# DocF/multispectral-object-detection

Measured on AMD Instinct MI355X. Metric: image-pairs/sec fwd, yolov5l+CFTx3 640×640 bs64, 1/2/4/8 GPU, higher is better.
Workload: dtype bf16; 1 GPU; cfg3 (yolov5l_fusion_transformerx3_FLIR_aligned) two-stream forward, 640x640, 64 pairs/GPU, BN folded, pre-NMS detections; pairs_per_gpu=64, image_size=640, parallelism=batch-shard x1, hip_graph=True, two_hip_streams=False, forwards_in_flight=3, streams_per_forward_in_flight=1, single_in_flight_streams=2

## Files before the change

### multispectral-object-detection_amd/csrc/attention.hip

```cpp
#include "cft_common.h"

template <typename T>
__global__ void __launch_bounds__(256) attention_kernel(const unsigned char* __restrict__ qkv, unsigned char* __restrict__ out,
                                                        int heads, int dkp, float scale, uint32_t drop_thresh, float inv_keep,
                                                        unsigned long long seed) {
  constexpr int GE = Elem<T>::GE;
  constexpr int ES = (int)sizeof(T);
  constexpr int T_TOK = 128;
  constexpr int KT = GE / 4;
  constexpr int NCH = 8 / KT;
  constexpr int PS_B = T_TOK * ES + 16;
  extern __shared__ __attribute__((aligned(16))) unsigned char smem[];
  const int KS_B = dkp * ES + 16;
  unsigned char* sK = smem;
  unsigned char* sVT = smem + T_TOK * KS_B;

  const int b = blockIdx.x / heads, head = blockIdx.x % heads;
  const int tid = threadIdx.x, lane = tid & 63, wave = tid >> 6;
  const int lrow = lane & 15, lgrp = lane >> 4;
  const int G = dkp / GE;
  const long ldq_b = (long)3 * heads * dkp * ES;
  const long ldo_b = (long)heads * dkp * ES;
  const unsigned char* qbase = qkv + (long)b * T_TOK * ldq_b + (long)head * dkp * ES;
  const unsigned char* kbase = qbase + (long)heads * dkp * ES;
  const unsigned char* vbase = kbase + (long)heads * dkp * ES;

#define ATT_STAGE_VT(c0_, cw_)                                                                             \
  {                                                                                                        \
    const int cg_ = (cw_) / GE;                                                                            \
    for (int i = tid; i < T_TOK * cg_; i += 256) {                                                         \
      const int t = i / cg_, kg = i - t * cg_;                                                             \
      const gran_t g = *reinterpret_cast<const gran_t*>(vbase + t * ldq_b + (long)((c0_) + kg * GE) * ES); \
      if (ES == 2) {                                                                                       \
        _Pragma("unroll") for (int e = 0; e < 4; ++e) {                                                    \
          *reinterpret_cast<uint16_t*>(sVT + (kg * GE + 2 * e) * PS_B + t * 2) = (uint16_t)(g[e] & 0xffffu); \
          *reinterpret_cast<uint16_t*>(sVT + (kg * GE + 2 * e + 1) * PS_B + t * 2) = (uint16_t)(g[e] >> 16); \
        }                                                                                                  \
      } else {                                                                                             \
        _Pragma("unroll") for (int e = 0; e < 4; ++e)                                                      \
          *reinterpret_cast<uint32_t*>(sVT + (kg * GE + e) * PS_B + t * 4) = g[e];                         \
      }                                                                                                    \
    }                                                                                                      \
  }

  for (int i = tid; i < T_TOK * G; i += 256) {
    const int t = i / G, kg = i - t * G;
    *reinterpret_cast<gran_t*>(sK + t * KS_B + kg * 16) = *reinterpret_cast<const gran_t*>(kbase + t * ldq_b + kg * 16);
  }
  {
    const int cw0 = dkp < 64 ? dkp : 64;
    ATT_STAGE_VT(0, cw0)
  }
  __syncthreads();

  f32x4_t s[2][8];
#pragma unroll
  for (int i = 0; i < 2; ++i)
#pragma unroll
    for (int j = 0; j < 8; ++j) s[i][j] = f32x4_t{0.f, 0.f, 0.f, 0.f};
  const int ksteps = G >> 2;
  for (int ks = 0; ks < ksteps; ++ks) {
    const int kg = ks * 4 + lgrp;
    gran_t qf[2];
#pragma unroll
    for (int i = 0; i < 2; ++i)
      qf[i] = *reinterpret_cast<const gran_t*>(qbase + (long)(wave * 32 + i * 16 + lrow) * ldq_b + kg * 16);
#pragma unroll
    for (int j = 0; j < 8; ++j) {
      const gran_t kf = *reinterpret_cast<const gran_t*>(sK + (j * 16 + lrow) * KS_B + kg * 16);
#pragma unroll
      for (int i = 0; i < 2; ++i) s[i][j] = mma_granule<T>(kf, qf[i], s[i][j]);
    }
  }

  float inv_sum[2];
  gran_t pf[2][NCH];
#pragma unroll
  for (int i = 0; i < 2; ++i) {
    float mx = -INFINITY;
#pragma unroll
    for (int j = 0; j < 8; ++j)
#pragma unroll
      for (int e = 0; e < 4; ++e) { s[i][j][e] *= scale; mx = fmaxf(mx, s[i][j][e]); }
    mx = fmaxf(mx, __shfl_xor(mx, 16));
    mx = fmaxf(mx, __shfl_xor(mx, 32));
    float sum = 0.f;
#pragma unroll
    for (int j = 0; j < 8; ++j)
#pragma unroll
      for (int e = 0; e < 4; ++e) { const float pv = __expf(s[i][j][e] - mx); s[i][j][e] = pv; sum += pv; }
    sum += __shfl_xor(sum, 16);
    sum += __shfl_xor(sum, 32);
    inv_sum[i] = 1.0f / sum;
    if (drop_thresh != 0u) {
      const unsigned long long qrow = ((unsigned long long)blockIdx.x * T_TOK + (wave * 32 + i * 16 + lrow)) * T_TOK;
#pragma unroll
      for (int j = 0; j < 8; ++j)
#pragma unroll
        for (int e = 0; e < 4; ++e)
          s[i][j][e] = cft_hash32(seed, qrow + (unsigned)(j * 16 + lgrp * 4 + e)) >= drop_thresh ? s[i][j][e] * inv_keep : 0.0f;
    }
#pragma unroll
    for (int c = 0; c < NCH; ++c) {
      if constexpr (ES == 2) {
        typedef Elem<typename Half16<T>::type> E16;
        pf[i][c] = gran_t{E16::pack2(s[i][2 * c][0], s[i][2 * c][1]), E16::pack2(s[i][2 * c][2], s[i][2 * c][3]),
                          E16::pack2(s[i][2 * c + 1][0], s[i][2 * c + 1][1]), E16::pack2(s[i][2 * c + 1][2], s[i][2 * c + 1][3])};
      } else {
        pf[i][c] = gran_t{__float_as_uint(s[i][c][0]), __float_as_uint(s[i][c][1]), __float_as_uint(s[i][c][2]), __float_as_uint(s[i][c][3])};
      }
    }
  }

  for (int c0 = 0; c0 < dkp; c0 += 64) {
    const int cw = (dkp - c0) < 64 ? (dkp - c0) : 64;
    if (c0 > 0) {
      __syncthreads();
      ATT_STAGE_VT(c0, cw)
      __syncthreads();
    }
    const int ntc = cw >> 4;
    f32x4_t o[2][4];
#pragma unroll
    for (int i = 0; i < 2; ++i)
#pragma unroll
      for (int j = 0; j < 4; ++j) o[i][j] = f32x4_t{0.f, 0.f, 0.f, 0.f};
#pragma unroll
    for (int c = 0; c < NCH; ++c) {
#pragma unroll
      for (int j = 0; j < 4; ++j) {
        if (j < ntc) {
          const unsigned char* vrow = sVT + (j * 16 + lrow) * PS_B;
          gran_t vf;
          if constexpr (ES == 2) {
            const uint2 lo = *reinterpret_cast<const uint2*>(vrow + ((2 * c) * 16 + lgrp * 4) * 2);
            const uint2 hi = *reinterpret_cast<const uint2*>(vrow + ((2 * c + 1) * 16 + lgrp * 4) * 2);
            vf = gran_t{lo.x, lo.y, hi.x, hi.y};
          } else {
            vf = *reinterpret_cast<const gran_t*>(vrow + (c * 16 + lgrp * 4) * 4);
          }
#pragma unroll
          for (int i = 0; i < 2; ++i) o[i][j] = mma_granule<T>(vf, pf[i][c], o[i][j]);
        }
      }
    }
#pragma unroll
    for (int i = 0; i < 2; ++i)
#pragma unroll
      for (int j = 0; j < 4; ++j) {
        if (j < ntc) {
          const int row = wave * 32 + i * 16 + lrow;
          float v[4];
#pragma unroll
          for (int e = 0; e < 4; ++e) v[e] = o[i][j][e] * inv_sum[i];
          unsigned char* dst = out + ((long)b * T_TOK + row) * ldo_b + ((long)head * dkp + c0 + j * 16 + lgrp * 4) * ES;
          if constexpr (ES == 2) {
            typedef Elem<typename Half16<T>::type> E16;
            *reinterpret_cast<uint2*>(dst) = uint2{E16::pack2(v[0], v[1]), E16::pack2(v[2], v[3])};
          }
          else *reinterpret_cast<f32x4_t*>(dst) = f32x4_t{v[0], v[1], v[2], v[3]};
        }
      }
  }
#undef ATT_STAGE_VT
}

extern "C" int cft_attention(const void* qkv, void* out, int B, int heads, int dk, int dkp,
                             int dtype, float attn_pdrop, unsigned long long seed, void* stream) {
  CFT_REQUIRE(qkv && out, "cft_attention: null pointer");
  CFT_REQUIRE(attn_pdrop >= 0.0f && attn_pdrop < 1.0f, "cft_attention: attn_pdrop must be in [0, 1) (0 = inference)");
  CFT_REQUIRE(cft_is_dtype(dtype), "cft_attention: bad dtype");
  const int es = cft_elem_size(dtype);
  const int kstep = es == 2 ? 32 : 16;
  CFT_REQUIRE(B > 0 && heads > 0 && dk > 0 && dkp >= dk && dkp % kstep == 0 && dkp <= 256, "cft_attention: dkp must be a multiple of 32 (bf16, f16) / 16 (f32), >= dk, <= 256");
  const int ps = 128 * es + 16, ks = dkp * es + 16;
  const size_t smem = (size_t)128 * ks + (size_t)64 * ps;
  CFT_REQUIRE(smem <= 160 * 1024, "cft_attention: head too wide for LDS");
  const float scale = 1.0f / sqrtf((float)dk);
  CFT_DISPATCH_DTYPE(dtype, T, {
    cft_allow_lds<&attention_kernel<T>>(160 * 1024);
    hipLaunchKernelGGL(attention_kernel<T>, dim3(B * heads), dim3(256), smem, as_stream(stream), (const unsigned char*)qkv, (unsigned char*)out, heads, dkp, scale,
                       (uint32_t)((double)attn_pdrop * 4294967296.0), 1.0f / (1.0f - attn_pdrop), seed);
  });
  return cft_check_launch("attention_kernel");
}
```

### multispectral-object-detection_amd/csrc/pointwise.hip

```cpp
#include "cft_common.h"
#include "resize_common.h"

static inline int grid_for(long work, int block) {
  long g = (work + block - 1) / block;
  const long cap = 256L * 16;
  return (int)(g < 1 ? 1 : (g > cap ? cap : g));
}

template <typename T>
__global__ void __launch_bounds__(256) focus_s2d_kernel(const float* __restrict__ in, unsigned char* __restrict__ out,
                                                        int B, int H, int W) {
  const int Ho = H >> 1, Wo = W >> 1;
  const long total = (long)B * Ho * Wo;
  for (long idx = (long)blockIdx.x * blockDim.x + threadIdx.x; idx < total; idx += (long)gridDim.x * blockDim.x) {
    const int x = (int)(idx % Wo);
    const long t = idx / Wo;
    const int y = (int)(t % Ho);
    const int b = (int)(t / Ho);
    float v[16];
#pragma unroll
    for (int c = 0; c < 3; ++c) {
      const float* base = in + (((long)b * 3 + c) * H + 2 * y) * W + 2 * x;
      const float2 top = *reinterpret_cast<const float2*>(base);
      const float2 bot = *reinterpret_cast<const float2*>(base + W);
      v[0 + c] = top.x;
      v[3 + c] = bot.x;
      v[6 + c] = top.y;
      v[9 + c] = bot.y;
    }
    v[12] = v[13] = v[14] = v[15] = 0.f;
    constexpr int GE = Elem<T>::GE;
    gran_t* o = reinterpret_cast<gran_t*>(out + idx * 16 * sizeof(T));
#pragma unroll
    for (int k = 0; k < 16 / GE; ++k) o[k] = Elem<T>::pack(v + k * GE);
  }
}

extern "C" int cft_focus_s2d(const float* in, void* out, int B, int H, int W, int dtype, void* stream) {
  CFT_REQUIRE(in && out, "cft_focus_s2d: null pointer");
  CFT_REQUIRE(B > 0 && H > 0 && W > 0 && (H % 2 == 0) && (W % 2 == 0), "cft_focus_s2d: H and W must be even");
  CFT_REQUIRE(cft_is_dtype(dtype), "cft_focus_s2d: bad dtype");
  const long total = (long)B * (H / 2) * (W / 2);
  const int grid = grid_for(total, 256);
  CFT_DISPATCH_DTYPE(dtype, T, hipLaunchKernelGGL(focus_s2d_kernel<T>, dim3(grid), dim3(256), 0, as_stream(stream), in, (unsigned char*)out, B, H, W));
  return cft_check_launch("focus_s2d_kernel");
}

template <typename T>
__global__ void __launch_bounds__(256) focus_s2d_u8_kernel(const unsigned char* __restrict__ in, long sb, long sc, long sh,
                                                           unsigned char* __restrict__ out, int B, int H, int W, float scale) {
  const int Ho = H >> 1, Wo = W >> 1;
  const long total = (long)B * Ho * Wo;
  for (long idx = (long)blockIdx.x * blockDim.x + threadIdx.x; idx < total; idx += (long)gridDim.x * blockDim.x) {
    const int x = (int)(idx % Wo);
    const long t = idx / Wo;
    const int y = (int)(t % Ho);
    const int b = (int)(t / Ho);
    float v[16];
#pragma unroll
    for (int c = 0; c < 3; ++c) {
      const unsigned char* base = in + (long)b * sb + (long)c * sc + (long)(2 * y) * sh + 2 * x;
      v[0 + c] = (float)base[0] * scale;
      v[6 + c] = (float)base[1] * scale;
      v[3 + c] = (float)base[sh] * scale;
      v[9 + c] = (float)base[sh + 1] * scale;
    }
    v[12] = v[13] = v[14] = v[15] = 0.f;
    constexpr int GE = Elem<T>::GE;
    gran_t* o = reinterpret_cast<gran_t*>(out + idx * 16 * sizeof(T));
#pragma unroll
    for (int k = 0; k < 16 / GE; ++k) o[k] = Elem<T>::pack(v + k * GE);
  }
}

extern "C" int cft_focus_s2d_u8(const unsigned char* in, long stride_b, long stride_c, long stride_h, void* out,
                                int B, int H, int W, float scale, int dtype, void* stream) {
  CFT_REQUIRE(in && out, "cft_focus_s2d_u8: null pointer");
  CFT_REQUIRE(B > 0 && H > 0 && W > 0 && (H % 2 == 0) && (W % 2 == 0), "cft_focus_s2d_u8: H and W must be even");
  CFT_REQUIRE(cft_is_dtype(dtype), "cft_focus_s2d_u8: bad dtype");
  CFT_REQUIRE(stride_h >= W && stride_c > 0 && stride_b > 0, "cft_focus_s2d_u8: bad strides");
  const long total = (long)B * (H / 2) * (W / 2);
  const int grid = grid_for(total, 256);
  CFT_DISPATCH_DTYPE(dtype, T, hipLaunchKernelGGL(focus_s2d_u8_kernel<T>, dim3(grid), dim3(256), 0, as_stream(stream), in, stride_b, stride_c, stride_h, (unsigned char*)out, B, H, W, scale));
  return cft_check_launch("focus_s2d_u8_kernel");
}

template <typename T>
__device__ __forceinline__ void gmax(float* a, const gran_t& g) {
  float f[Elem<T>::GE];
  Elem<T>::unpack(g, f);
// ... 15 lines not shown
  const long pix_stride = (long)ld * sizeof(T);
  for (int i = threadIdx.x; i < HW; i += blockDim.x) plane[i] = *reinterpret_cast<const gran_t*>(base + i * pix_stride);
  __syncthreads();
  const int rad[3] = {r1, r2, r3};
  for (int i = threadIdx.x; i < HW; i += blockDim.x) {
    const int y = i / W, x = i - y * W;
    float m[GE];
#pragma unroll
    for (int e = 0; e < GE; ++e) m[e] = -INFINITY;
    int done = -1;
#pragma unroll
    for (int k = 0; k < 3; ++k) {
      for (int d = done + 1; d <= rad[k]; ++d) {
        if (d == 0) { gmax<T>(m, plane[i]); continue; }
        if (x - d >= 0) gmax<T>(m, plane[i - d]);
        if (x + d < W) gmax<T>(m, plane[i + d]);
      }
      done = rad[k];
      rowm[k * HW + i] = Elem<T>::pack(m);
    }
  }
  __syncthreads();
  for (int i = threadIdx.x; i < HW; i += blockDim.x) {
    const int y = i / W;
#pragma unroll
    for (int k = 0; k < 3; ++k) {
      float m[GE];
#pragma unroll
      for (int e = 0; e < GE; ++e) m[e] = -INFINITY;
      const gran_t* src = rowm + k * HW;
      for (int d = -rad[k]; d <= rad[k]; ++d)
        if ((unsigned)(y + d) < (unsigned)H) gmax<T>(m, src[i + d * W]);
      *reinterpret_cast<gran_t*>(base + i * pix_stride + (long)(k + 1) * C * sizeof(T)) = Elem<T>::pack(m);
    }
  }
}

template <typename T>
__global__ void __launch_bounds__(512) spp_chain_kernel(unsigned char* buf, int H, int W, int C, int ld, int r, int G) {
  constexpr int GE = Elem<T>::GE;
  extern __shared__ __attribute__((aligned(16))) unsigned char smem[];
  const int HW = H * W, n = HW * G;
  gran_t* A = reinterpret_cast<gran_t*>(smem);
  gran_t* Bp = A + n;
  const int groups = (C / GE) / G;
  const int b = blockIdx.x / groups, g0 = (blockIdx.x - b * groups) * G;
  unsigned char* base = buf + ((long)b * HW * ld + (long)g0 * GE) * sizeof(T);
  const long pix_stride = (long)ld * sizeof(T);
  for (int i = threadIdx.x; i < n; i += blockDim.x) {
    const int px = i / G, g = i - px * G;
    A[i] = *reinterpret_cast<const gran_t*>(base + px * pix_stride + g * 16);
  }
  __syncthreads();
  for (int k = 0; k < 3; ++k) {
    for (int i = threadIdx.x; i < n; i += blockDim.x) {
      const int px = i / G;
      const int x = px % W;
      float m[GE];
      Elem<T>::unpack(A[i], m);
      for (int d = 1; d <= r; ++d) {
        if (x - d >= 0) gmax<T>(m, A[i - d * G]);
        if (x + d < W) gmax<T>(m, A[i + d * G]);
      }
      Bp[i] = Elem<T>::pack(m);
    }
    __syncthreads();
    for (int i = threadIdx.x; i < n; i += blockDim.x) {
      const int px = i / G, g = i - px * G;
      const int y = px / W;
      float m[GE];
      Elem<T>::unpack(Bp[i], m);
      for (int d = 1; d <= r; ++d) {
        if (y - d >= 0) gmax<T>(m, Bp[i - d * W * G]);
        if (y + d < H) gmax<T>(m, Bp[i + d * W * G]);
      }
      const gran_t o = Elem<T>::pack(m);
      A[i] = o;
      *reinterpret_cast<gran_t*>(base + px * pix_stride + ((long)(k + 1) * C * sizeof(T)) + g * 16) = o;
    }
    __syncthreads();
  }
}

extern "C" int cft_spp_maxpool(void* buf, int B, int H, int W, int C, int ld, int k1, int k2, int k3,
                               int dtype, void* stream) {
  CFT_REQUIRE(buf != nullptr, "cft_spp_maxpool: null pointer");
  CFT_REQUIRE(cft_is_dtype(dtype), "cft_spp_maxpool: bad dtype");
  const int ge = cft_granule(dtype);
  CFT_REQUIRE(C % ge == 0 && ld % ge == 0 && ld >= 4 * C, "cft_spp_maxpool: C/ld not granule aligned or ld < 4C");
  CFT_REQUIRE((k1 & 1) && (k2 & 1) && (k3 & 1) && k1 <= k2 && k2 <= k3 && k3 <= 13 && k1 >= 1, "cft_spp_maxpool: kernel sizes must be odd, ascending, <= 13");
  const int r1 = k1 / 2, r2 = k2 / 2, r3 = k3 / 2, gpc = C / ge;
  if (r1 >= 1 && r2 == 2 * r1 && r3 == 3 * r1 && (size_t)2 * H * W * 16 <= 160 * 1024) {
    int G = 1;
    for (int g = 4; g > 1; g >>= 1)
      if (gpc % g == 0 && (size_t)2 * H * W * g * 16 <= 64 * 1024) { G = g; break; }
    const size_t smem = (size_t)2 * H * W * G * 16;
    const int grid = B * (gpc / G);
    CFT_DISPATCH_DTYPE(dtype, T, {
      cft_allow_lds<&spp_chain_kernel<T>>(160 * 1024);
      hipLaunchKernelGGL(spp_chain_kernel<T>, dim3(grid), dim3(512), smem, as_stream(stream), (unsigned char*)buf, H, W, C, ld, r1, G);
    });
    return cft_check_launch("spp_chain_kernel");
  }
  const size_t smem = (size_t)4 * H * W * 16;
  CFT_REQUIRE(smem <= 160 * 1024, "cft_spp_maxpool: feature map too large for the LDS plane (H*W <= 2560)");
  const int grid = B * gpc;
  CFT_DISPATCH_DTYPE(dtype, T, {
    cft_allow_lds<&spp_maxpool_kernel<T>>(160 * 1024);
    hipLaunchKernelGGL(spp_maxpool_kernel<T>, dim3(grid), dim3(256), smem, as_stream(stream), (unsigned char*)buf, H, W, C, ld, r1, r2, r3);
  });
  return cft_check_launch("spp_maxpool_kernel");
}

__global__ void __launch_bounds__(256) copy_channels_kernel(const unsigned char* __restrict__ in, long ldi_b, long ioff_b,
                                                            unsigned char* __restrict__ out, long ldo_b, long ooff_b,
                                                            int B, int Ho, int Wo, int gpp, int up) {
  const long total = (long)B * Ho * Wo * gpp;
  const int Hi = Ho >> up, Wi = Wo >> up;
  for (long idx = (long)blockIdx.x * blockDim.x + threadIdx.x; idx < total; idx += (long)gridDim.x * blockDim.x) {
    const int gidx = (int)(idx % gpp);
    long t = idx / gpp;
    const int x = (int)(t % Wo); t /= Wo;
    const int y = (int)(t % Ho);
    const int b = (int)(t / Ho);
    const long ipix = ((long)b * Hi + (y >> up)) * Wi + (x >> up);
    const long opix = ((long)b * Ho + y) * Wo + x;
    *reinterpret_cast<gran_t*>(out + opix * ldo_b + ooff_b + gidx * 16L) =
        *reinterpret_cast<const gran_t*>(in + ipix * ldi_b + ioff_b + gidx * 16L);
  }
}

extern "C" int cft_copy_channels(const void* in, int ldi, int ioff, void* out, int ldo, int ooff,
                                 int B, int Ho, int Wo, int C, int up, int dtype, void* stream) {
  CFT_REQUIRE(in && out, "cft_copy_channels: null pointer");
  CFT_REQUIRE(cft_is_dtype(dtype), "cft_copy_channels: bad dtype");
  const int ge = cft_granule(dtype), es = cft_elem_size(dtype);
  CFT_REQUIRE(C % ge == 0 && ldi % ge == 0 && ioff % ge == 0 && ldo % ge == 0 && ooff % ge == 0, "cft_copy_channels: not granule aligned");
  CFT_REQUIRE(up >= 0 && up <= 3 && (Ho % (1 << up) == 0) && (Wo % (1 << up) == 0), "cft_copy_channels: bad upsample shift");
  const int gpp = C / ge;
  const long total = (long)B * Ho * Wo * gpp;
  hipLaunchKernelGGL(copy_channels_kernel, dim3(grid_for(total, 256)), dim3(256), 0, as_stream(stream),
                     (const unsigned char*)in, (long)ldi * es, (long)ioff * es, (unsigned char*)out, (long)ldo * es, (long)ooff * es,
                     B, Ho, Wo, gpp, up);
  return cft_check_launch("copy_channels_kernel");
}

template <typename TI, typename TO>
__global__ void __launch_bounds__(256) to_nhwc_kernel(const unsigned char* __restrict__ in, long sb, long sc, long sh, long sw,
                                                      unsigned char* __restrict__ out, long ldo_b, long ooff_b,
                                                      int B, int C, int H, int W, int gpp) {
  constexpr int GE = Elem<TO>::GE;
  const long total = (long)B * H * W * gpp;
  for (long idx = (long)blockIdx.x * blockDim.x + threadIdx.x; idx < total; idx += (long)gridDim.x * blockDim.x) {
    const int gidx = (int)(idx % gpp);
    long t = idx / gpp;
    const int x = (int)(t % W); t /= W;
    const int y = (int)(t % H);
    const int b = (int)(t / H);
    float v[GE];
#pragma unroll
    for (int e = 0; e < GE; ++e) {
      const int c = gidx * GE + e;
      float f = 0.0f;
      if (c < C) {
        const long o = (long)b * sb + (long)c * sc + (long)y * sh + (long)x * sw;
        if constexpr (sizeof(TI) == 4) f = reinterpret_cast<const float*>(in)[o];
        else {
          float lo, hi;
          Elem<TI>::unpack2((uint32_t)reinterpret_cast<const uint16_t*>(in)[o], lo, hi);
          f = lo;
        }
      }
      v[e] = f;
    }
    *reinterpret_cast<gran_t*>(out + (((long)b * H + y) * W + x) * ldo_b + ooff_b + gidx * 16L) = Elem<TO>::pack(v);
  }
}

extern "C" int cft_to_nhwc(const void* in, int in_dtype, long stride_b, long stride_c, long stride_h, long stride_w,
                           void* out, int ldo, int ooff, int B, int C, int cpad, int H, int W, int dtype, void* stream) {
// ... 5 lines not shown
  CFT_REQUIRE(ldo % ge == 0 && ooff % ge == 0 && ldo >= ooff + cpad, "cft_to_nhwc: output ld/offset not granule aligned or too small");
  const int gpp = cpad / ge;
  const long total = (long)B * H * W * gpp;
  const int grid = grid_for(total, 256);
  CFT_DISPATCH_DTYPE(in_dtype, TI, CFT_DISPATCH_DTYPE(dtype, TO,
      hipLaunchKernelGGL((to_nhwc_kernel<TI, TO>), dim3(grid), dim3(256), 0, as_stream(stream), (const unsigned char*)in, stride_b, stride_c, stride_h, stride_w,
                         (unsigned char*)out, (long)ldo * es, (long)ooff * es, B, C, H, W, gpp)));
  return cft_check_launch("to_nhwc_kernel");
}

template <typename T>
__global__ void __launch_bounds__(256) add_kernel(const unsigned char* a, long lda_b, long aoff_b,
                                                  const unsigned char* b, long ldb_b, long boff_b,
                                                  unsigned char* out, long ldo_b, long ooff_b, long M, int gpp) {
  constexpr int GE = Elem<T>::GE;
  const long total = M * gpp;
  for (long idx = (long)blockIdx.x * blockDim.x + threadIdx.x; idx < total; idx += (long)gridDim.x * blockDim.x) {
    const long m = idx / gpp;
    const long go = (idx - m * gpp) * 16L;
    float fa[GE], fb[GE];
    Elem<T>::unpack(*reinterpret_cast<const gran_t*>(a + m * lda_b + aoff_b + go), fa);
    Elem<T>::unpack(*reinterpret_cast<const gran_t*>(b + m * ldb_b + boff_b + go), fb);
#pragma unroll
    for (int e = 0; e < GE; ++e) fa[e] += fb[e];
    *reinterpret_cast<gran_t*>(out + m * ldo_b + ooff_b + go) = Elem<T>::pack(fa);
  }
}

extern "C" int cft_add(const void* a, int lda, int aoff, const void* b, int ldb, int boff,
                       void* out, int ldo, int ooff, long M, int C, int dtype, void* stream) {
  CFT_REQUIRE(a && b && out, "cft_add: null pointer");
  CFT_REQUIRE(cft_is_dtype(dtype), "cft_add: bad dtype");
  const int ge = cft_granule(dtype), es = cft_elem_size(dtype);
  CFT_REQUIRE(C % ge == 0 && lda % ge == 0 && aoff % ge == 0 && ldb % ge == 0 && boff % ge == 0 && ldo % ge == 0 && ooff % ge == 0,
              "cft_add: not granule aligned");
  const int gpp = C / ge;
  const int grid = grid_for(M * gpp, 256);
  CFT_DISPATCH_DTYPE(dtype, T, hipLaunchKernelGGL(add_kernel<T>, dim3(grid), dim3(256), 0, as_stream(stream), (const unsigned char*)a, (long)lda * es, (long)aoff * es,
                                                   (const unsigned char*)b, (long)ldb * es, (long)boff * es, (unsigned char*)out, (long)ldo * es, (long)ooff * es, M, gpp));
  return cft_check_launch("add_kernel");
}

static int cft_fail(const char* who, const char* what) {
  char buf[256];
  snprintf(buf, sizeof(buf), "%s: %s", who, what);
  cft_set_error(buf);
  return CFT_EINVAL;
}
#define CFT_REQUIRE_WHO(cond, what) \
  do {                              \
    if (!(cond)) return cft_fail(who, what); \
  } while (0)

#define CFT_GRID_RULE "anchor grid must satisfy 1 <= va, ha and va * ha <= 1024"
static inline bool cft_grid_ok(int va, int ha) { return va >= 1 && ha >= 1 && va * ha <= 1024; }

struct ChanRef {
  const void* p;
  int ld, off;
  bool aligned(int ge) const { return p == nullptr || (ld % ge == 0 && off % ge == 0); }
  unsigned char* ptr() const { return (unsigned char*)p; }
};

template <typename T, int VA, int HA>
__global__ void __launch_bounds__(256) gpt_tokenize_kernel(const unsigned char* rgb, long ld_rgb_b, long off_rgb_b,
                                                           const unsigned char* ir, long ld_ir_b, long off_ir_b,
                                                           const float* __restrict__ pos_emb, float* __restrict__ tokens,
                                                           int H, int W, int C, int va_arg, int ha_arg) {
  constexpr int GE = Elem<T>::GE;
  const int va = VA ? VA : va_arg, ha = HA ? HA : ha_arg;
  const int ncell = va * ha, ntok = 2 * ncell;
  const int b = blockIdx.x / ntok, cell = blockIdx.x - b * ntok;
  const int s = cell >= ncell ? 1 : 0, r = cell - s * ncell;
  const int i = r / ha, j = r - i * ha;
  const int h0 = (i * H) / va, h1 = ((i + 1) * H + va - 1) / va;
  const int w0 = (j * W) / ha, w1 = ((j + 1) * W + ha - 1) / ha;
  const unsigned char* src = s ? ir : rgb;
  const long ldb = s ? ld_ir_b : ld_rgb_b, offb = s ? off_ir_b : off_rgb_b;
  const float inv = 1.0f / (float)((h1 - h0) * (w1 - w0));
  for (int cg = threadIdx.x; cg < C / GE; cg += blockDim.x) {
    float acc[GE];
#pragma unroll
    for (int e = 0; e < GE; ++e) acc[e] = 0.f;
    for (int y = h0; y < h1; ++y)
      for (int x = w0; x < w1; ++x) {
        float f[GE];
        Elem<T>::unpack(*reinterpret_cast<const gran_t*>(src + (((long)b * H + y) * W + x) * ldb + offb + cg * 16L), f);
#pragma unroll
        for (int e = 0; e < GE; ++e) acc[e] += f[e];
      }
    float* o = tokens + ((long)b * ntok + cell) * C + cg * GE;
    const float* pe = pos_emb + (long)cell * C + cg * GE;
#pragma unroll
    for (int e = 0; e < GE; ++e) o[e] = acc[e] * inv + pe[e];
  }
}

template <int VA, int HA>
static int gpt_tokenize_launch(const char* who, ChanRef rgb, ChanRef ir, const float* pos_emb, float* tokens,
                               int B, int H, int W, int C, int va, int ha, int dtype, void* stream) {
  CFT_REQUIRE_WHO(rgb.p && ir.p && pos_emb && tokens, "null pointer");
  CFT_REQUIRE_WHO(cft_is_dtype(dtype), "bad dtype");
  const int ge = cft_granule(dtype);
  const long es = cft_elem_size(dtype);
  CFT_REQUIRE_WHO(C % ge == 0 && rgb.aligned(ge) && ir.aligned(ge), "not granule aligned");
  CFT_REQUIRE_WHO(B > 0 && H >= 1 && W >= 1, "bad shape");
  if constexpr (VA == 0) {
    CFT_REQUIRE_WHO(cft_grid_ok(va, ha), CFT_GRID_RULE);
    CFT_REQUIRE_WHO((long)B * 2 * va * ha < (1L << 31), "too many tokens");
  }
  int threads = C / ge;
  threads = threads < 64 ? 64 : (threads > 256 ? 256 : ((threads + 63) / 64) * 64);
  CFT_DISPATCH_DTYPE(dtype, T, hipLaunchKernelGGL((gpt_tokenize_kernel<T, VA, HA>), dim3(B * 2 * va * ha), dim3(threads), 0, as_stream(stream),
                                                   rgb.ptr(), rgb.ld * es, rgb.off * es, ir.ptr(), ir.ld * es, ir.off * es, pos_emb, tokens, H, W, C, va, ha));
  return cft_check_launch("gpt_tokenize_kernel");
}

extern "C" int cft_gpt_tokenize(const void* rgb, int ld_rgb, int off_rgb, const void* ir, int ld_ir, int off_ir,
                                const float* pos_emb, float* tokens, int B, int H, int W, int C,
                                int dtype, void* stream) {
  return gpt_tokenize_launch<8, 8>("cft_gpt_tokenize", {rgb, ld_rgb, off_rgb}, {ir, ld_ir, off_ir}, pos_emb, tokens, B, H, W, C, 8, 8, dtype, stream);
}

extern "C" int cft_gpt_tokenize_grid(const void* rgb, int ld_rgb, int off_rgb, const void* ir, int ld_ir, int off_ir,
                                     const float* pos_emb, float* tokens, int B, int H, int W, int C, int va, int ha,
                                     int dtype, void* stream) {
  return gpt_tokenize_launch<0, 0>("cft_gpt_tokenize_grid", {rgb, ld_rgb, off_rgb}, {ir, ld_ir, off_ir}, pos_emb, tokens, B, H, W, C, va, ha, dtype, stream);
}

template <int MAXV, bool REDUCE>
__global__ void __launch_bounds__(256) layernorm_kernel(float* __restrict__ x, const float* __restrict__ gamma, const float* __restrict__ beta,
                                                        unsigned char* __restrict__ y, long rows, int C, float eps, int out_dtype,
                                                        const float* __restrict__ parts, int nparts, long part_stride) {
  const int lane = threadIdx.x & 63;
  const long row = (long)blockIdx.x * 4 + (threadIdx.x >> 6);
  if (row >= rows) return;
  const int nv = C >> 2;
  float4* xr = reinterpret_cast<float4*>(x + row * C);
  float4 v[MAXV];
  float s = 0.f;
#pragma unroll
  for (int k = 0; k < MAXV; ++k) {
    const int idx = lane + k * 64;
    v[k] = make_float4(0.f, 0.f, 0.f, 0.f);
    if (idx < nv) {
      float4 a = xr[idx];
      if constexpr (REDUCE) {
        for (int sp = 0; sp < nparts; ++sp) {
          const float4 q = reinterpret_cast<const float4*>(parts + sp * part_stride + row * C)[idx];
          a.x += q.x; a.y += q.y; a.z += q.z; a.w += q.w;
        }
        xr[idx] = a;
      }
      v[k] = a;
    }
    s += v[k].x + v[k].y + v[k].z + v[k].w;
  }
#pragma unroll
  for (int o = 32; o > 0; o >>= 1) s += __shfl_xor(s, o);
  const float mean = s / (float)C;
  float q = 0.f;
#pragma unroll
  for (int k = 0; k < MAXV; ++k) {
    const int idx = lane + k * 64;
    if (idx < nv) {
      const float a = v[k].x - mean, b = v[k].y - mean, c = v[k].z - mean, d = v[k].w - mean;
      q += a * a + b * b + c * c + d * d;
    }
  }
#pragma unroll
  for (int o = 32; o > 0; o >>= 1) q += __shfl_xor(q, o);
  const float rstd = rsqrtf(q / (float)C + eps);
#pragma unroll
// ... 115 lines not shown
          for (int e = 0; e < GE; ++e) v0[e] += v1[e];
          *reinterpret_cast<gran_t*>(sum + pix * lds_b + soff_b + cb) = Elem<T>::pack(v0);
        }
      } else {
#pragma unroll
        for (int e = 0; e < GE; ++e) v0[e] += hx * r0[e] + lx * r1[e];
        *reinterpret_cast<gran_t*>(out0 + pix * ldo0_b + ooff0_b + cb) = Elem<T>::pack(v0);
      }
    }
  }
}

static inline int gpt_upsample_grid_chunk(int C, int ha, int ns) {
  int cw = (16 * 1024) / (ns * ha);
  cw -= cw % 8;
  return C < cw ? C : cw;
}

template <bool DUAL, int VA, int HA>
static int gpt_upsample_launch(const char* who, const float* tokens, int s, ChanRef base0, ChanRef base1, ChanRef out0, ChanRef out1, ChanRef sum,
                               int B, int H, int W, int C, int va, int ha, int dtype, void* stream) {
  constexpr int NS = DUAL ? 2 : 1;
  const int ge = cft_granule(dtype);
  const long es = cft_elem_size(dtype);
  CFT_REQUIRE_WHO(C % ge == 0 && base0.aligned(ge) && base1.aligned(ge) && out0.aligned(ge) && out1.aligned(ge) && sum.aligned(ge), "not granule aligned");
  int cw = C;
  if constexpr (VA != 0) {
    CFT_REQUIRE_WHO(C % 4 == 0 && (long)B * H < (1L << 31), "C must be a multiple of 4");
    CFT_REQUIRE_WHO((size_t)NS * HA * C * sizeof(float) <= (size_t)NS * 64 * 1024,
                    DUAL ? "C too large for the LDS rows (C <= 2048)" : "C too large for the LDS row (C <= 2048)");
  } else {
    CFT_REQUIRE_WHO(C % 4 == 0 && C <= 2048 && B > 0 && H >= 1 && W >= 1 && (long)B * H < (1L << 31), "C must be a multiple of 4, <= 2048");
    cw = gpt_upsample_grid_chunk(C, ha, NS);
  }
  const size_t smem = (size_t)NS * ha * cw * sizeof(float);
  CFT_DISPATCH_DTYPE(dtype, T, {
    if constexpr (DUAL && VA != 0) cft_allow_lds<&gpt_upsample_kernel<T, DUAL, VA, HA>>(128 * 1024);
    hipLaunchKernelGGL((gpt_upsample_kernel<T, DUAL, VA, HA>), dim3(B * H), dim3(256), smem, as_stream(stream), tokens, s,
                       base0.ptr(), base0.ld * es, base0.off * es, base1.ptr(), base1.ld * es, base1.off * es,
                       out0.ptr(), out0.ld * es, out0.off * es, out1.ptr(), out1.ld * es, out1.off * es,
                       sum.ptr(), sum.ld * es, sum.off * es, B, H, W, C, va, ha, cw);
  });
  return cft_check_launch("gpt_upsample_kernel");
}

extern "C" int cft_gpt_upsample_add(const float* tokens, int s, const void* base, int ldb, int boff,
                                    void* out, int ldo, int ooff, int B, int H, int W, int C,
                                    int dtype, void* stream) {
  CFT_REQUIRE(tokens && out, "cft_gpt_upsample_add: null pointer");
  CFT_REQUIRE(cft_is_dtype(dtype), "cft_gpt_upsample_add: bad dtype");
  CFT_REQUIRE(s == 0 || s == 1, "cft_gpt_upsample_add: stream index must be 0 or 1");
  return gpt_upsample_launch<false, 8, 8>("cft_gpt_upsample_add", tokens, s, {base, ldb, boff}, {}, {out, ldo, ooff}, {}, {}, B, H, W, C, 8, 8, dtype, stream);
}

extern "C" int cft_gpt_upsample_add2(const float* tokens, const void* base0, int ldb0, int boff0, const void* base1, int ldb1, int boff1,
                                     void* out0, int ldo0, int ooff0, void* out1, int ldo1, int ooff1, void* sum, int lds, int soff,
                                     int B, int H, int W, int C, int dtype, void* stream) {
  CFT_REQUIRE(tokens && base0 && base1 && out0 && out1, "cft_gpt_upsample_add2: null pointer");
  CFT_REQUIRE(cft_is_dtype(dtype), "cft_gpt_upsample_add2: bad dtype");
  return gpt_upsample_launch<true, 8, 8>("cft_gpt_upsample_add2", tokens, 0, {base0, ldb0, boff0}, {base1, ldb1, boff1}, {out0, ldo0, ooff0},
                                         {out1, ldo1, ooff1}, {sum, lds, soff}, B, H, W, C, 8, 8, dtype, stream);
}

extern "C" int cft_gpt_upsample_add_grid(const float* tokens, int s, const void* base, int ldb, int boff,
                                         void* out, int ldo, int ooff, int B, int H, int W, int C, int va, int ha,
                                         int dtype, void* stream) {
  CFT_REQUIRE(tokens && out, "cft_gpt_upsample_add_grid: null pointer");
  CFT_REQUIRE(cft_is_dtype(dtype), "cft_gpt_upsample_add_grid: bad dtype");
  CFT_REQUIRE(s == 0 || s == 1, "cft_gpt_upsample_add_grid: stream index must be 0 or 1");
  CFT_REQUIRE(cft_grid_ok(va, ha), "cft_gpt_upsample_add_grid: " CFT_GRID_RULE);
  return gpt_upsample_launch<false, 0, 0>("cft_gpt_upsample_add_grid", tokens, s, {base, ldb, boff}, {}, {out, ldo, ooff}, {}, {}, B, H, W, C, va, ha, dtype, stream);
}

extern "C" int cft_gpt_upsample_add2_grid(const float* tokens, const void* base0, int ldb0, int boff0, const void* base1, int ldb1, int boff1,
                                          void* out0, int ldo0, int ooff0, void* out1, int ldo1, int ooff1, void* sum, int lds, int soff,
                                          int B, int H, int W, int C, int va, int ha, int dtype, void* stream) {
  CFT_REQUIRE(tokens && base0 && base1 && out0 && out1, "cft_gpt_upsample_add2_grid: null pointer");
  CFT_REQUIRE(cft_is_dtype(dtype), "cft_gpt_upsample_add2_grid: bad dtype");
  CFT_REQUIRE(cft_grid_ok(va, ha), "cft_gpt_upsample_add2_grid: " CFT_GRID_RULE);
  return gpt_upsample_launch<true, 0, 0>("cft_gpt_upsample_add2_grid", tokens, 0, {base0, ldb0, boff0}, {base1, ldb1, boff1}, {out0, ldo0, ooff0},
                                         {out1, ldo1, ooff1}, {sum, lds, soff}, B, H, W, C, va, ha, dtype, stream);
}

__global__ void __launch_bounds__(256) detect_decode_kernel(const float* __restrict__ logits, int ldl, float* __restrict__ raw,
                                                            float* __restrict__ pred, const float* __restrict__ anchors,
                                                            int B, int ny, int nx, int na, int no, float stride,
                                                            long row0, long total_rows) {
  const long total = (long)B * na * ny * nx * no;
  for (long idx = (long)blockIdx.x * blockDim.x + threadIdx.x; idx < total; idx += (long)gridDim.x * blockDim.x) {
    const int o = (int)(idx % no);
    long t = idx / no;
    const int x = (int)(t % nx); t /= nx;
    const int y = (int)(t % ny); t /= ny;
    const int a = (int)(t % na);
    const int b = (int)(t / na);
    const float v = logits[(((long)b * ny + y) * nx + x) * ldl + a * no + o];
    raw[idx] = v;
    const float sg = 1.0f / (1.0f + __expf(-v));
    float r;
    if (o == 0) r = (sg * 2.0f - 0.5f + (float)x) * stride;
    else if (o == 1) r = (sg * 2.0f - 0.5f + (float)y) * stride;
    else if (o < 4) { const float w = sg * 2.0f; r = w * w * anchors[a * 2 + (o - 2)]; }
    else r = sg;
    pred[((long)b * total_rows + row0 + ((long)a * ny + y) * nx + x) * no + o] = r;
  }
}

extern "C" int cft_detect_decode(const float* logits, int ldl, float* raw, float* pred, const float* anchors,
                                 int B, int ny, int nx, int na, int no, float stride,
                                 long row0, long total_rows, void* stream) {
  CFT_REQUIRE(logits && raw && pred && anchors, "cft_detect_decode: null pointer");
  CFT_REQUIRE(B > 0 && ny > 0 && nx > 0 && na > 0 && no >= 5 && ldl >= na * no, "cft_detect_decode: bad shape");
  CFT_REQUIRE(row0 >= 0 && row0 + (long)na * ny * nx <= total_rows, "cft_detect_decode: rows out of range");
  const long total = (long)B * na * ny * nx * no;
  hipLaunchKernelGGL(detect_decode_kernel, dim3(grid_for(total, 256)), dim3(256), 0, as_stream(stream), logits, ldl, raw, pred, anchors,
                     B, ny, nx, na, no, stride, row0, total_rows);
  return cft_check_launch("detect_decode_kernel");
}

__global__ void __launch_bounds__(256) letterbox_u8_kernel(const unsigned char* __restrict__ src, int sh, int sw, long src_row_stride,
                                                           unsigned char* __restrict__ dst, int dh, int dw, long dsy, long dsx, long dsc, int flip,
                                                           int rh, int rw, int top, int left, int c0, int c1, int c2) {
  const long total = (long)dh * dw;
  const double scale_x = cft_linear_scale(rw, sw), scale_y = cft_linear_scale(rh, sh);
  const bool resize = rh != sh || rw != sw;
  for (long idx = (long)blockIdx.x * blockDim.x + threadIdx.x; idx < total; idx += (long)gridDim.x * blockDim.x) {
    const int y = (int)(idx / dw), x = (int)(idx - (long)y * dw);
    const int ry = y - top, rx = x - left;
    int v[3] = {c0, c1, c2};
    if (ry >= 0 && ry < rh && rx >= 0 && rx < rw) {
      if (!resize) {
        const unsigned char* s = src + (long)ry * src_row_stride + rx * 3L;
        v[0] = s[0]; v[1] = s[1]; v[2] = s[2];
      } else {
        const CftLinearTap tx = cft_linear_tap_x(rx, scale_x, sw), ty = cft_linear_tap_y(ry, scale_y, sh);
        const unsigned char* r0 = src + (long)ty.s0 * src_row_stride;
        const unsigned char* r1 = src + (long)ty.s1 * src_row_stride;
#pragma unroll
        for (int c = 0; c < 3; ++c)
          v[c] = cft_linear_blend(r0[tx.s0 * 3 + c], r0[tx.s1 * 3 + c], r1[tx.s0 * 3 + c], r1[tx.s1 * 3 + c], tx, ty);
      }
    }
#pragma unroll
    for (int c = 0; c < 3; ++c) {
      int o = v[c];
      o = o < 0 ? 0 : (o > 255 ? 255 : o);
      dst[(long)y * dsy + (long)x * dsx + (long)(flip ? 2 - c : c) * dsc] = (unsigned char)o;
    }
  }
}

extern "C" int cft_letterbox_u8(const unsigned char* src, int src_h, int src_w, long src_row_stride,
                                unsigned char* dst, int dst_h, int dst_w, long dst_stride_y, long dst_stride_x, long dst_stride_c, int flip_channels,
                                int resized_h, int resized_w, int top, int left, int color0, int color1, int color2, void* stream) {
  CFT_REQUIRE(src && dst, "cft_letterbox_u8: null pointer");
  CFT_REQUIRE(src_h > 0 && src_w > 0 && dst_h > 0 && dst_w > 0 && resized_h > 0 && resized_w > 0, "cft_letterbox_u8: non-positive size");
  CFT_REQUIRE(top >= 0 && left >= 0 && top + resized_h <= dst_h && left + resized_w <= dst_w, "cft_letterbox_u8: the resized image does not fit the destination");
  CFT_REQUIRE(src_row_stride >= 3L * src_w, "cft_letterbox_u8: bad source row stride");
  const long total = (long)dst_h * dst_w;
  hipLaunchKernelGGL(letterbox_u8_kernel, dim3(grid_for(total, 256)), dim3(256), 0, as_stream(stream), src, src_h, src_w, src_row_stride,
                     dst, dst_h, dst_w, dst_stride_y, dst_stride_x, dst_stride_c, flip_channels, resized_h, resized_w, top, left, color0, color1, color2);
  return cft_check_launch("letterbox_u8_kernel");
}
```

Measured before the change: 3702 image-pairs/sec.

## Specialize attention staging, add SPP r2 kernel, vectorize detect decode and pooling

Measured after the change: 3722 image-pairs/sec, median of 5. About the same (+0.6%).

```diff
diff --git a/multispectral-object-detection_amd/csrc/attention.hip b/multispectral-object-detection_amd/csrc/attention.hip
--- a/multispectral-object-detection_amd/csrc/attention.hip
+++ b/multispectral-object-detection_amd/csrc/attention.hip
@@ -1,6 +1,6 @@
 #include "cft_common.h"
 
-template <typename T>
+template <typename T, int GC>
 __global__ void __launch_bounds__(256) attention_kernel(const unsigned char* __restrict__ qkv, unsigned char* __restrict__ out,
                                                         int heads, int dkp, float scale, uint32_t drop_thresh, float inv_keep,
                                                         unsigned long long seed) {
@@ -18,12 +18,28 @@
   const int b = blockIdx.x / heads, head = blockIdx.x % heads;
   const int tid = threadIdx.x, lane = tid & 63, wave = tid >> 6;
   const int lrow = lane & 15, lgrp = lane >> 4;
-  const int G = dkp / GE;
+  const int G = GC ? GC : dkp / GE;
+  constexpr int CG0 = GC * GE < 64 ? GC : 64 / GE;
+  constexpr int KIT = GC / 2, VIT = CG0 / 2;
+  constexpr int QST = GC / 4;
   const long ldq_b = (long)3 * heads * dkp * ES;
   const long ldo_b = (long)heads * dkp * ES;
   const unsigned char* qbase = qkv + (long)b * T_TOK * ldq_b + (long)head * dkp * ES;
   const unsigned char* kbase = qbase + (long)heads * dkp * ES;
   const unsigned char* vbase = kbase + (long)heads * dkp * ES;
+
+#define ATT_SCATTER_VT(g_, t_, kg_)                                                                          \
+  {                                                                                                          \
+    if (ES == 2) {                                                                                           \
+      _Pragma("unroll") for (int e = 0; e < 4; ++e) {                                                        \
+        *reinterpret_cast<uint16_t*>(sVT + ((kg_) * GE + 2 * e) * PS_B + (t_) * 2) = (uint16_t)((g_)[e] & 0xffffu); \
+        *reinterpret_cast<uint16_t*>(sVT + ((kg_) * GE + 2 * e + 1) * PS_B + (t_) * 2) = (uint16_t)((g_)[e] >> 16); \
+      }                                                                                                      \
+    } else {                                                                                                 \
+      _Pragma("unroll") for (int e = 0; e < 4; ++e)                                                          \
+        *reinterpret_cast<uint32_t*>(sVT + ((kg_) * GE + e) * PS_B + (t_) * 4) = (g_)[e];                    \
+    }                                                                                                        \
+  }
 
 #define ATT_STAGE_VT(c0_, cw_)                                                                             \
   {                                                                                                        \
@@ -31,27 +47,55 @@
     for (int i = tid; i < T_TOK * cg_; i += 256) {                                                         \
       const int t = i / cg_, kg = i - t * cg_;                                                             \
       const gran_t g = *reinterpret_cast<const gran_t*>(vbase + t * ldq_b + (long)((c0_) + kg * GE) * ES); \
-      if (ES == 2) {                                                                                       \
-        _Pragma("unroll") for (int e = 0; e < 4; ++e) {                                                    \
-          *reinterpret_cast<uint16_t*>(sVT + (kg * GE + 2 * e) * PS_B + t * 2) = (uint16_t)(g[e] & 0xffffu); \
-          *reinterpret_cast<uint16_t*>(sVT + (kg * GE + 2 * e + 1) * PS_B + t * 2) = (uint16_t)(g[e] >> 16); \
-        }                                                                                                  \
-      } else {                                                                                             \
-        _Pragma("unroll") for (int e = 0; e < 4; ++e)                                                      \
-          *reinterpret_cast<uint32_t*>(sVT + (kg * GE + e) * PS_B + t * 4) = g[e];                         \
-      }                                                                                                    \
+      ATT_SCATTER_VT(g, t, kg)                                                                             \
     }                                                                                                      \
   }
 
-  for (int i = tid; i < T_TOK * G; i += 256) {
-    const int t = i / G, kg = i - t * G;
-    *reinterpret_cast<gran_t*>(sK + t * KS_B + kg * 16) = *reinterpret_cast<const gran_t*>(kbase + t * ldq_b + kg * 16);
-  }
-  {
+  gran_t qr[GC ? QST : 1][2];
+  gran_t vn[GC ? VIT : 1];
+  if constexpr (GC != 0) {
+    gran_t kr[KIT];
+#pragma unroll
+    for (int it = 0; it < KIT; ++it) {
+      const int i = tid + it * 256, t = i / GC, kg = i % GC;
+      kr[it] = *reinterpret_cast<const gran_t*>(kbase + t * ldq_b + kg * 16);
+    }
+#pragma unroll
+    for (int it = 0; it < VIT; ++it) {
+      const int i = tid + it * 256, t = i / CG0, kg = i % CG0;
+      vn[it] = *reinterpret_cast<const gran_t*>(vbase + t * ldq_b + (long)(kg * GE) * ES);
+    }
+#pragma unroll
+    for (int ks = 0; ks < QST; ++ks)
+#pragma unroll
+      for (int i = 0; i < 2; ++i)
+        qr[ks][i] = *reinterpret_cast<const gran_t*>(qbase + (long)(wave * 32 + i * 16 + lrow) * ldq_b + (ks * 4 + lgrp) * 16);
+#pragma unroll
+    for (int it = 0; it < KIT; ++it) {
+      const int i = tid + it * 256, t = i / GC, kg = i % GC;
+      *reinterpret_cast<gran_t*>(sK + t * KS_B + kg * 16) = kr[it];
+    }
+#pragma unroll
+    for (int it = 0; it < VIT; ++it) {
+      const int i = tid + it * 256, t = i / CG0, kg = i % CG0;
+      ATT_SCATTER_VT(vn[it], t, kg)
+    }
+  } else {
+    for (int i = tid; i < T_TOK * G; i += 256) {
+      const int t = i / G, kg = i - t * G;
+      *reinterpret_cast<gran_t*>(sK + t * KS_B + kg * 16) = *reinterpret_cast<const gran_t*>(kbase + t * ldq_b + kg * 16);
+    }
     const int cw0 = dkp < 64 ? dkp : 64;
     ATT_STAGE_VT(0, cw0)
   }
   __syncthreads();
+  if constexpr (GC * GE > 64) {
+#pragma unroll
+    for (int it = 0; it < VIT; ++it) {
+      const int i = tid + it * 256, t = i / CG0, kg = i % CG0;
+      vn[it] = *reinterpret_cast<const gran_t*>(vbase + t * ldq_b + (long)(64 + kg * GE) * ES);
+    }
+  }
 
   f32x4_t s[2][8];
 #pragma unroll
@@ -59,12 +103,15 @@
 #pragma unroll
     for (int j = 0; j < 8; ++j) s[i][j] = f32x4_t{0.f, 0.f, 0.f, 0.f};
   const int ksteps = G >> 2;
+#pragma unroll
   for (int ks = 0; ks < ksteps; ++ks) {
     const int kg = ks * 4 + lgrp;
     gran_t qf[2];
 #pragma unroll
-    for (int i = 0; i < 2; ++i)
-      qf[i] = *reinterpret_cast<const gran_t*>(qbase + (long)(wave * 32 + i * 16 + lrow) * ldq_b + kg * 16);
+    for (int i = 0; i < 2; ++i) {
+      if constexpr (GC != 0) qf[i] = qr[ks][i];
+      else qf[i] = *reinterpret_cast<const gran_t*>(qbase + (long)(wave * 32 + i * 16 + lrow) * ldq_b + kg * 16);
+    }
 #pragma unroll
     for (int j = 0; j < 8; ++j) {
       const gran_t kf = *reinterpret_cast<const gran_t*>(sK + (j * 16 + lrow) * KS_B + kg * 16);
@@ -116,7 +163,15 @@
     const int cw = (dkp - c0) < 64 ? (dkp - c0) : 64;
     if (c0 > 0) {
       __syncthreads();
-      ATT_STAGE_VT(c0, cw)
+      if constexpr (GC != 0) {
+#pragma unroll
+        for (int it = 0; it < VIT; ++it) {
+          const int i = tid + it * 256, t = i / CG0, kg = i % CG0;
+          ATT_SCATTER_VT(vn[it], t, kg)
+        }
+      } else {
+        ATT_STAGE_VT(c0, cw)
+      }
       __syncthreads();
     }
     const int ntc = cw >> 4;
@@ -163,6 +218,7 @@
       }
   }
 #undef ATT_STAGE_VT
+#undef ATT_SCATTER_VT
 }
 
 extern "C" int cft_attention(const void* qkv, void* out, int B, int heads, int dk, int dkp,
@@ -177,10 +233,22 @@
   const size_t smem = (size_t)128 * ks + (size_t)64 * ps;
   CFT_REQUIRE(smem <= 160 * 1024, "cft_attention: head too wide for LDS");
   const float scale = 1.0f / sqrtf((float)dk);
+  const int G = dkp / cft_granule(dtype);
+  const auto launch = [&](auto kernel) {
+    hipLaunchKernelGGL(kernel, dim3(B * heads), dim3(256), smem, as_stream(stream), (const unsigned char*)qkv, (unsigned char*)out, heads, dkp, scale,
+                       (uint32_t)((double)attn_pdrop * 4294967296.0), 1.0f / (1.0f - attn_pdrop), seed);
+  };
+#define ATT_LAUNCH(GC_)                                        \
+  {                                                            \
+    cft_allow_lds<&attention_kernel<T, GC_>>(160 * 1024);      \
+    launch(attention_kernel<T, GC_>);                          \
+  }
   CFT_DISPATCH_DTYPE(dtype, T, {
-    cft_allow_lds<&attention_kernel<T>>(160 * 1024);
-    hipLaunchKernelGGL(attention_kernel<T>, dim3(B * heads), dim3(256), smem, as_stream(stream), (const unsigned char*)qkv, (unsigned char*)out, heads, dkp, scale,
-                       (uint32_t)((double)attn_pdrop * 4294967296.0), 1.0f / (1.0f - attn_pdrop), seed);
+    if (G == 4) ATT_LAUNCH(4)
+    else if (G == 8) ATT_LAUNCH(8)
+    else if (G == 16) ATT_LAUNCH(16)
+    else ATT_LAUNCH(0)
   });
+#undef ATT_LAUNCH
   return cft_check_launch("attention_kernel");
 }
diff --git a/multispectral-object-detection_amd/csrc/pointwise.hip b/multispectral-object-detection_amd/csrc/pointwise.hip
--- a/multispectral-object-detection_amd/csrc/pointwise.hip
+++ b/multispectral-object-detection_amd/csrc/pointwise.hip
@@ -6,6 +6,18 @@
   const long cap = 256L * 16;
   return (int)(g < 1 ? 1 : (g > cap ? cap : g));
 }
+
+struct Recip {
+  uint32_t mul, sh;
+};
+static Recip recip_of(int d) {
+  if (d <= 1) return {0u, 0u};
+  int l = 0;
+  while ((1L << l) < d) ++l;
+  const unsigned long long k = 31ULL + l;
+  return {(uint32_t)(((1ULL << k) / (unsigned long long)d) + 1ULL), (uint32_t)(k - 32)};
+}
+__device__ __forceinline__ int rdiv(int n, Recip r) { return r.mul ? (int)(__umulhi((uint32_t)n, r.mul) >> r.sh) : n; }
 
 template <typename T>
 __global__ void __launch_bounds__(256) focus_s2d_kernel(const float* __restrict__ in, unsigned char* __restrict__ out,
@@ -187,6 +199,70 @@
   }
 }
 
+template <typename T>
+__global__ void __launch_bounds__(512) spp_chain_kernel_r2(unsigned char* buf, int H, int W, int C, int ld, int gs, Recip rw) {
+  constexpr int GE = Elem<T>::GE;
+  constexpr int NI = 4;
+  extern __shared__ __attribute__((aligned(16))) unsigned char smem[];
+  const int G = 1 << gs;
+  const int HW = H * W, n = HW * G;
+  gran_t* A = reinterpret_cast<gran_t*>(smem);
+  gran_t* Bp = A + n;
+  const int groups = (C / GE) >> gs;
+  const int b = blockIdx.x / groups, g0 = (blockIdx.x - b * groups) << gs;
+  unsigned char* base = buf + ((long)b * HW * ld + (long)g0 * GE) * sizeof(T);
+  const long pix_stride = (long)ld * sizeof(T);
+  const long pool_stride = (long)C * sizeof(T);
+  int li[NI], edge[NI];
+  gran_t v[NI];
+#pragma unroll
+  for (int k = 0; k < NI; ++k) {
+    const int i = threadIdx.x + k * 512;
+    li[k] = i < n ? i : n - 1;
+    const int px = li[k] >> gs, g = li[k] - (px << gs);
+    const int y = rdiv(px, rw), x = px - y * W;
+    const int xl = x < 2 ? x : 2, xr = W - 1 - x < 2 ? W - 1 - x : 2, yu = y < 2 ? y : 2, yd = H - 1 - y < 2 ? H - 1 - y : 2;
+    edge[k] = xl | xr << 2 | yu << 4 | yd << 6;
+    v[k] = *reinterpret_cast<const gran_t*>(base + px * pix_stride + g * 16);
+  }
+#pragma unroll
+  for (int k = 0; k < NI; ++k)
+    if (threadIdx.x + k * 512 < n) A[li[k]] = v[k];
+  __syncthreads();
+  const int WG = W << gs;
+  for (int p = 0; p < 3; ++p) {
+#pragma unroll
+    for (int k = 0; k < NI; ++k) {
+      const int i = li[k], xl = edge[k] & 3, xr = (edge[k] >> 2) & 3;
+      float m[GE];
+      Elem<T>::unpack(A[i], m);
+      gmax<T>(m, A[i - (xl >= 1 ? G : 0)]);
+      gmax<T>(m, A[i + (xr >= 1 ? G : 0)]);
+      gmax<T>(m, A[i - (xl >= 2 ? 2 * G : 0)]);
+      gmax<T>(m, A[i + (xr >= 2 ? 2 * G : 0)]);
+      if (threadIdx.x + k * 512 < n) Bp[i] = Elem<T>::pack(m);
+    }
+    __syncthreads();
+#pragma unroll
+    for (int k = 0; k < NI; ++k) {
+      const int i = li[k], yu = (edge[k] >> 4) & 3, yd = (edge[k] >> 6) & 3;
+      float m[GE];
+      Elem<T>::unpack(Bp[i], m);
+      gmax<T>(m, Bp[i - (yu >= 1 ? WG : 0)]);
+      gmax<T>(m, Bp[i + (yd >= 1 ? WG : 0)]);
+      gmax<T>(m, Bp[i - (yu >= 2 ? 2 * WG : 0)]);
+      gmax<T>(m, Bp[i + (yd >= 2 ? 2 * WG : 0)]);
+      if (threadIdx.x + k * 512 < n) {
+        const gran_t o = Elem<T>::pack(m);
+        const int px = i >> gs, g = i - (px << gs);
+        A[i] = o;
+        *reinterpret_cast<gran_t*>(base + px * pix_stride + (p + 1) * pool_stride + g * 16) = o;
+      }
+    }
+    __syncthreads();
+  }
+}
+
 extern "C" int cft_spp_maxpool(void* buf, int B, int H, int W, int C, int ld, int k1, int k2, int k3,
                                int dtype, void* stream) {
   CFT_REQUIRE(buf != nullptr, "cft_spp_maxpool: null pointer");
@@ -201,6 +277,14 @@
       if (gpc % g == 0 && (size_t)2 * H * W * g * 16 <= 64 * 1024) { G = g; break; }
     const size_t smem = (size_t)2 * H * W * G * 16;
     const int grid = B * (gpc / G);
+    if (r1 == 2 && H * W * G <= 4 * 512) {
+      const int gs = G == 4 ? 2 : (G == 2 ? 1 : 0);
+      CFT_DISPATCH_DTYPE(dtype, T, {
+        cft_allow_lds<&spp_chain_kernel_r2<T>>(160 * 1024);
+        hipLaunchKernelGGL(spp_chain_kernel_r2<T>, dim3(grid), dim3(512), smem, as_stream(stream), (unsigned char*)buf, H, W, C, ld, gs, recip_of(W));
+      });
+      return cft_check_launch("spp_chain_kernel_r2");
+    }
     CFT_DISPATCH_DTYPE(dtype, T, {
       cft_allow_lds<&spp_chain_kernel<T>>(160 * 1024);
       hipLaunchKernelGGL(spp_chain_kernel<T>, dim3(grid), dim3(512), smem, as_stream(stream), (unsigned char*)buf, H, W, C, ld, r1, G);
@@ -372,13 +456,31 @@
     float acc[GE];
 #pragma unroll
     for (int e = 0; e < GE; ++e) acc[e] = 0.f;
-    for (int y = h0; y < h1; ++y)
-      for (int x = w0; x < w1; ++x) {
-        float f[GE];
-        Elem<T>::unpack(*reinterpret_cast<const gran_t*>(src + (((long)b * H + y) * W + x) * ldb + offb + cg * 16L), f);
-#pragma unroll
-        for (int e = 0; e < GE; ++e) acc[e] += f[e];
-      }
+    constexpr int NB = 8;
+    const int ww = w1 - w0, nwin = (h1 - h0) * ww;
+    int y = h0, x = w0;
+    for (int p0 = 0; p0 < nwin; p0 += NB) {
+      gran_t g[NB];
+      int yy = y, xx = x;
+#pragma unroll
+      for (int k = 0; k < NB; ++k) {
+        g[k] = *reinterpret_cast<const gran_t*>(src + (((long)b * H + yy) * W + xx) * ldb + offb + cg * 16L);
+        xx += p0 + k + 1 < nwin ? 1 : 0;
+        const bool wrap = xx == w1;
+        xx = wrap ? w0 : xx;
+        yy += wrap ? 1 : 0;
+      }
+#pragma unroll
+      for (int k = 0; k < NB; ++k) {
+        if (p0 + k < nwin) {
+          float f[GE];
+          Elem<T>::unpack(g[k], f);
+#pragma unroll
+          for (int e = 0; e < GE; ++e) acc[e] += f[e];
+        }
+      }
+      y = yy; x = xx;
+    }
     float* o = tokens + ((long)b * ntok + cell) * C + cg * GE;
     const float* pe = pos_emb + (long)cell * C + cg * GE;
 #pragma unroll
@@ -660,18 +762,31 @@
                                          {out1, ldo1, ooff1}, {sum, lds, soff}, B, H, W, C, va, ha, dtype, stream);
 }
 
+struct DecodeRecips {
+  Recip no, nx, ny, na;
+};
+template <bool WIDE>
 __global__ void __launch_bounds__(256) detect_decode_kernel(const float* __restrict__ logits, int ldl, float* __restrict__ raw,
                                                             float* __restrict__ pred, const float* __restrict__ anchors,
                                                             int B, int ny, int nx, int na, int no, float stride,
-                                                            long row0, long total_rows) {
+                                                            long row0, long total_rows, DecodeRecips rc) {
   const long total = (long)B * na * ny * nx * no;
   for (long idx = (long)blockIdx.x * blockDim.x + threadIdx.x; idx < total; idx += (long)gridDim.x * blockDim.x) {
-    const int o = (int)(idx % no);
-    long t = idx / no;
-    const int x = (int)(t % nx); t /= nx;
-    const int y = (int)(t % ny); t /= ny;
-    const int a = (int)(t % na);
-    const int b = (int)(t / na);
+    int o, x, y, a, b;
+    if constexpr (WIDE) {
+      o = (int)(idx % no);
+      long t = idx / no;
+      x = (int)(t % nx); t /= nx;
+      y = (int)(t % ny); t /= ny;
+      a = (int)(t % na);
+      b = (int)(t / na);
+    } else {
+      int t = rdiv((int)idx, rc.no), q;
+      o = (int)idx - t * no;
+      q = rdiv(t, rc.nx); x = t - q * nx; t = q;
+      q = rdiv(t, rc.ny); y = t - q * ny; t = q;
+      b = rdiv(t, rc.na); a = t - b * na;
+    }
     const float v = logits[(((long)b * ny + y) * nx + x) * ldl + a * no + o];
     raw[idx] = v;
     const float sg = 1.0f / (1.0f + __expf(-v));
@@ -684,6 +799,48 @@
   }
 }
 
+template <int NQ>
+__global__ void __launch_bounds__(256) detect_decode_kernel_rows(const float* __restrict__ logits, int ldl, float* __restrict__ raw,
+                                                                 float* __restrict__ pred, const float* __restrict__ anchors,
+                                                                 int B, int ny, int nx, int na, int no, float stride,
+                                                                 long row0, long total_rows, DecodeRecips rc) {
+  const int rows = B * na * ny * nx;
+  const int nq = NQ ? NQ : no >> 2;
+  for (int r = blockIdx.x * blockDim.x + threadIdx.x; r < rows; r += gridDim.x * blockDim.x) {
+    const int pix = rdiv(r, rc.na), a = r - pix * na;
+    const int t = rdiv(pix, rc.nx), x = pix - t * nx;
+    const int b = rdiv(t, rc.ny), y = t - b * ny;
+    const float4* src = reinterpret_cast<const float4*>(logits + (long)pix * ldl + a * no);
+    const long cell = ((long)a * ny + y) * nx + x;
+    float4* rw = reinterpret_cast<float4*>(raw + ((long)b * na * ny * nx + cell) * no);
+    float4* pd = reinterpret_cast<float4*>(pred + ((long)b * total_rows + row0 + cell) * no);
+    float4 v[NQ ? NQ : 1];
+    if constexpr (NQ != 0) {
+#pragma unroll
+      for (int q = 0; q < NQ; ++q) v[q] = src[q];
+    }
+#pragma unroll
+    for (int q = 0; q < nq; ++q) {
+      if constexpr (NQ == 0) v[0] = src[q];
+      const float4 f = v[NQ ? q : 0];
+      rw[q] = f;
+      const float in[4] = {f.x, f.y, f.z, f.w};
+      float out[4];
+#pragma unroll
+      for (int e = 0; e < 4; ++e) {
+        const float sg = 1.0f / (1.0f + __expf(-in[e]));
+        float res;
+        if (q == 0 && e == 0) res = (sg * 2.0f - 0.5f + (float)x) * stride;
+        else if (q == 0 && e == 1) res = (sg * 2.0f - 0.5f + (float)y) * stride;
+        else if (q == 0) { const float w = sg * 2.0f; res = w * w * anchors[a * 2 + (e - 2)]; }
+        else res = sg;
+        out[e] = res;
+      }
+      pd[q] = make_float4(out[0], out[1], out[2], out[3]);
+    }
+  }
+}
+
 extern "C" int cft_detect_decode(const float* logits, int ldl, float* raw, float* pred, const float* anchors,
                                  int B, int ny, int nx, int na, int no, float stride,
                                  long row0, long total_rows, void* stream) {
@@ -691,8 +848,23 @@
   CFT_REQUIRE(B > 0 && ny > 0 && nx > 0 && na > 0 && no >= 5 && ldl >= na * no, "cft_detect_decode: bad shape");
   CFT_REQUIRE(row0 >= 0 && row0 + (long)na * ny * nx <= total_rows, "cft_detect_decode: rows out of range");
   const long total = (long)B * na * ny * nx * no;
-  hipLaunchKernelGGL(detect_decode_kernel, dim3(grid_for(total, 256)), dim3(256), 0, as_stream(stream), logits, ldl, raw, pred, anchors,
-                     B, ny, nx, na, no, stride, row0, total_rows);
+  const DecodeRecips rc = {recip_of(no), recip_of(nx), recip_of(ny), recip_of(na)};
+  const auto launch = [&](auto kernel) {
+    hipLaunchKernelGGL(kernel, dim3(grid_for(total, 256)), dim3(256), 0, as_stream(stream), logits, ldl, raw, pred, anchors,
+                       B, ny, nx, na, no, stride, row0, total_rows, rc);
+  };
+  const bool vec = total < (1L << 31) && no % 4 == 0 && ldl % 4 == 0 && ((uintptr_t)logits | (uintptr_t)raw | (uintptr_t)pred) % 16 == 0;
+  if (vec) {
+    const auto launch_rows = [&](auto kernel) {
+      hipLaunchKernelGGL(kernel, dim3(grid_for(total / no, 256)), dim3(256), 0, as_stream(stream), logits, ldl, raw, pred, anchors,
+                         B, ny, nx, na, no, stride, row0, total_rows, rc);
+    };
+    if (no == 8) launch_rows(detect_decode_kernel_rows<2>);
+    else launch_rows(detect_decode_kernel_rows<0>);
+    return cft_check_launch("detect_decode_kernel_rows");
+  }
+  if (total < (1L << 31)) launch(detect_decode_kernel<false>);
+  else launch(detect_decode_kernel<true>);
   return cft_check_launch("detect_decode_kernel");
 }
 
```
